# mnastorg/PSI-GNN

Hardware: AMD Instinct MI355X
Metric: fixed-point edges/sec (E' x Broyden iterations/sec) on 1M-node Poisson mesh (higher is better)
Workload: dtype f32

## Files before the change

### psi-gnn_amd/csrc/solver.hip

```cpp
#include "vec_helpers.h"
#include "internal.h"
#include "solver_shapes.h"
#include <stdlib.h>
#include <math.h>
#include <algorithm>
#include <vector>

struct Status {
  int32_t n_iter;
  int32_t done;
  int32_t prot_break;
  int32_t stop_reason;
  int32_t lowest_step;
  int32_t cur;
  int32_t low;
  int32_t nxt;
  double lowest_rel, lowest_abs_at;
  double rel0;
  double abs0;
  int32_t lowest_step_abs;
  int32_t stop_abs;
  double s, beta;
};

#define RB 256
static_assert(shapes::THREADS == TB && sizeof(Status) == shapes::STATUS_BYTES, "solver_shapes.h sizes the launches and the status block");
struct psignn_broyden {
  const psignn_plan* plan = nullptr;
  int64_t M = 0;
  int seq_len = D;
  int thr = 0;
  int keep_trace = 0;
  shapes::BroydenShape shape;
  float* jpart = nullptr;
  float *U = nullptr, *V = nullptr;
  float* xbuf = nullptr;
  float* gbuf[2] = {nullptr, nullptr};
  float *upd = nullptr, *fx = nullptr, *fwork = nullptr;
  float* lwork = nullptr;
  int64_t lwork_floats = 0;
  float* nrm_part = nullptr;
  float* part2 = nullptr;
  int a_ready = 0, a_from = 0;
  float* parta = nullptr;
  float *h0p = nullptr, *prbp = nullptr, *nrmp = nullptr;
  float* part = nullptr;
  float* coef = nullptr;
  Status* st = nullptr;
  double *rel_trace = nullptr, *abs_trace = nullptr;
  Status* h_st = nullptr;
  size_t bytes = 0;
  int ext_iter = 0;
  int hist = 0;
  int stop_abs = 0;
  int64_t size_hint = 0;
  int plan_order = 1;
};

__global__ void k_init_status(Status* st, double* rel_trace, double* abs_trace, int thr, int stop_abs = 0) {
  if (threadIdx.x == 0 && blockIdx.x == 0) {
    st->abs0 = 0.0; st->lowest_step_abs = 0; st->stop_abs = stop_abs;
    st->n_iter = 0; st->done = 0; st->prot_break = 0; st->stop_reason = 0; st->lowest_step = 0;
    st->cur = 0; st->low = 0; st->nxt = 1;
    st->lowest_rel = 1e8; st->lowest_abs_at = 1e8; st->rel0 = 0.0; st->s = 0.0; st->beta = 0.0;
  }
  for (int i = blockIdx.x * blockDim.x + threadIdx.x; i < thr; i += gridDim.x * blockDim.x) {
    rel_trace[i] = 0.0;
    abs_trace[i] = 0.0;
  }
}

template <int VEC>
__global__ __launch_bounds__(TB) void k_begin(int64_t M, const float* __restrict__ x0, const float* __restrict__ fx0,
                                              float* __restrict__ xb, float* __restrict__ gx, float* __restrict__ upd) {
  int64_t e0 = elem0<VEC>();
  if (e0 >= M) return;
// ... 254 lines not shown
  for (int j = 0; j < k; ++j) {
    float u[VEC];
    float sa = 0.f;
    if (act) {
      ldv_stream<VEC>(U + (int64_t)j * ld, e0, M, u);
#pragma unroll
      for (int i = 0; i < VEC; ++i) sa = fmaf(dx[i], u[i], sa);
    }
    sa = wave_sum(sa);
    const int q = j & 63;
    if (lead) sh.v[0][wv][q] = sa;
    if (q == 63 || j == k - 1) {
      float* const rows[1] = {rowb + (j - q)};
      stash_flush<1>(sh, q + 1, rows);
    }
  }
}

template <int VEC>
__global__ __launch_bounds__(TB) void k_sweep_u1(int64_t M, int k, const Status* __restrict__ st, const float* __restrict__ U,
                                                 const float* __restrict__ dxv, float* __restrict__ part, int ldp, int64_t ld) {
  sweep_u1_body<VEC>(M, k, st, U, dxv, part, ldp, ld);
}
template <int VEC>
__global__ __launch_bounds__(TB) void k_sweep_u1_bf16(int64_t M, int k, const Status* __restrict__ st, const __bf16* __restrict__ U,
                                                      const float* __restrict__ dxv, float* __restrict__ part, int ldp, int64_t ld) {
  sweep_u1_body<VEC, __bf16>(M, k, st, U, dxv, part, ldp, ld);
}

__device__ __forceinline__ void reduce_a_check_body(Status* st, const float* __restrict__ part, int nrows, int ldp, int thr, int k,
                                                    float* __restrict__ coef, const float* __restrict__ nrm_part, int nn,
                                                    double* __restrict__ rel_trace, double* __restrict__ abs_trace,
                                                    double eps, int seq_len, int keep_trace, double* sh,
                                                    const float* __restrict__ parta = nullptr, int nrows4 = 0, int a_from = 1 << 30) {
  if (blockIdx.y == RA) {
    if (blockIdx.x == 0) check_block(st, nrm_part, nn, rel_trace, abs_trace, eps, thr, seq_len, keep_trace, sh);
    return;
  }
  const int done = st->done;
  const int j = blockIdx.x, r = blockIdx.y;
  if (j >= k) return;
  const float* col = j >= a_from ? parta + (j - a_from) : part + j;
  const int n = j >= a_from ? nrows4 : nrows;
  const int64_t stride = j >= a_from ? PARTA_LD : ldp;
  const int lo = (int)((int64_t)n * r / RA), hi = (int)((int64_t)n * (r + 1) / RA);
  const double s = block_sum_col(col + (int64_t)lo * stride, hi - lo, stride, sh);
  if (threadIdx.x == 0 && !done) coef[(3 + r) * thr + j] = (float)s;
}
__global__ __launch_bounds__(RB) void k_reduce_a_check(Status* st, const float* __restrict__ part, int nrows, int ldp, int thr, int k,
                                                       float* __restrict__ coef, const float* __restrict__ nrm_part, int nn,
                                                       double* __restrict__ rel_trace, double* __restrict__ abs_trace,
                                                       double eps, int seq_len, int keep_trace, const float* __restrict__ parta,
                                                       int nrows4, int a_from) {
  __shared__ double sh[RB];
  reduce_a_check_body(st, part, nrows, ldp, thr, k, coef, nrm_part, nn, rel_trace, abs_trace, eps, seq_len, keep_trace, sh, parta, nrows4, a_from);
}

template <int VEC, class P = float>
__device__ __forceinline__ void sweep_v_body(int64_t M, int k, const Status* __restrict__ st, P* __restrict__ V,
                                             const float* __restrict__ dxv, const float* __restrict__ dgv,
                                             const float* __restrict__ gv, const float* __restrict__ coef,
                                             float* __restrict__ part, int64_t pstride, int ldp, float* __restrict__ part2, int nblk, int64_t ld,
                                             int thr) {
  __shared__ PairStash<2> sh;
  if (__builtin_amdgcn_readfirstlane(st->done)) return;
  int64_t e0 = elem0<VEC>();
  float dg[VEC], g[VEC], av[VEC];
  const bool act = e0 < M;
  if (act) {
    ldv<VEC>(dxv, e0, M, av);
    ldv<VEC>(dgv, e0, M, dg);
    ldv<VEC>(gv, e0, M, g);
#pragma unroll
    for (int i = 0; i < VEC; ++i) dg[i] = g[i] - dg[i];
#pragma unroll
    for (int i = 0; i < VEC; ++i) av[i] = -av[i];
  } else {
#pragma unroll
    for (int i = 0; i < VEC; ++i) dg[i] = g[i] = av[i] = 0.f;
  }
  const int wv = threadIdx.x >> 6;
  const int lane = threadIdx.x & 63;
  const bool lead = lane == 0;
  float* rowb = part + (int64_t)blockIdx.x * ldp;
  float cw = 0.f;
  auto step = [&](const int j, const float* v) {
    const int q = j & 63;
    if (q == 0) {
// ... 289 lines not shown
  float ccv = 0.f, cbv = 0.f;
  if (lane < NK) {
    ccv = coef[thr + j_keep0 + lane];
    cbv = coef[2 * thr + j_keep0 + lane];
  }
  const float sv = rfl((float)st->s), beta = rfl((float)st->beta);
#pragma unroll
  for (int q = 0; q < NK; ++q) {
    const float cc = __builtin_bit_cast(float, __builtin_amdgcn_readlane(__builtin_bit_cast(int, ccv), q));
    const float cb = __builtin_bit_cast(float, __builtin_amdgcn_readlane(__builtin_bit_cast(int, cbv), q));
    a1[0] = fmaf(-cc, kp[q].x, a1[0]); a1[1] = fmaf(-cc, kp[q].y, a1[1]); a1[2] = fmaf(-cc, kp[q].z, a1[2]); a1[3] = fmaf(-cc, kp[q].w, a1[3]);
    a2[0] = fmaf(-cb, kp[q].x, a2[0]); a2[1] = fmaf(-cb, kp[q].y, a2[1]); a2[2] = fmaf(-cb, kp[q].z, a2[2]); a2[3] = fmaf(-cb, kp[q].w, a2[3]);
  }
#pragma unroll
  for (int i = 0; i < 4; ++i) {
    float q = a1[i] / sv;
    q = (q != q) ? 0.f : q;
    a1[i] = q;
    a2[i] = fmaf(-q, beta, a2[i]);
  }
  st4_so_stream(U + (int64_t)k * ld, off, make_float4(a1[0], a1[1], a1[2], a1[3]));
  st4_so(upd, off, make_float4(a2[0], a2[1], a2[2], a2[3]));
#pragma unroll
  for (int q = 0; q < NK; ++q) {
    float sa = fmaf(kp[q].x, a2[0], fmaf(kp[q].y, a2[1], fmaf(kp[q].z, a2[2], kp[q].w * a2[3])));
    sa = wave_sum(sa);
    if (lead) ua[q] = sa;
  }
  float sa = fmaf(a1[0], a2[0], fmaf(a1[1], a2[1], fmaf(a1[2], a2[2], a1[3] * a2[3])));
  sa = wave_sum(sa);
  if (lead) ua[NK] = sa;
}

template <int KB>
__device__ __forceinline__ void sweep_u2r_body(int64_t M, int k, const Status* __restrict__ st, float* __restrict__ U,
                                               float* __restrict__ upd, const float* __restrict__ dgv,
                                               const float* __restrict__ gv, const float* __restrict__ coef, int thr,
                                               float* __restrict__ part, int64_t ld, int j_keep0) {
  __shared__ float ua[TB / 64][PARTA_LD];
  if (__builtin_amdgcn_readfirstlane(st->done)) return;
  const int tid = threadIdx.x;
  const int64_t e0 = elem0<4>();
  const int wv = __builtin_amdgcn_readfirstlane(tid >> 6);
  const bool lead = (tid & 63) == 0;
  const int64_t wave_e0 = ((int64_t)blockIdx.x * TB + (int64_t)__builtin_amdgcn_readfirstlane(tid & ~63)) * 4;
  if (wave_e0 + 256 <= M) {
    uint32_t off = ((blockIdx.x * (uint32_t)TB + ((uint32_t)tid & ~63u)) * 4u + ((uint32_t)tid & 63u) * 4u) * 4u;
    asm volatile("" : "+v"(off));
    float a1[4], a2[4];
#define U2R_CASE(n, first) case (n): u2r_kept<(n) < 0 ? 0 : (n), first>(a1, a2, k, st, U, upd, dgv, gv, coef, thr, ua[wv], ld, j_keep0, off, lead); break;
    if (j_keep0 == 0) {
      switch (k) {
        U2R_CASE(KB - 8, true) U2R_CASE(KB - 7, true) U2R_CASE(KB - 6, true) U2R_CASE(KB - 5, true) U2R_CASE(KB - 4, true)
        U2R_CASE(KB - 3, true) U2R_CASE(KB - 2, true) U2R_CASE(KB - 1, true) U2R_CASE(KB, true)
        default: break;
      }
    } else {
      {
        const float4 x = ld4_so(upd, off), go = ld4_so(dgv, off), g = ld4_so(gv, off);
        a1[0] = x.x + (g.x - go.x); a1[1] = x.y + (g.y - go.y); a1[2] = x.z + (g.z - go.z); a1[3] = x.w + (g.w - go.w);
        a2[0] = g.x; a2[1] = g.y; a2[2] = g.z; a2[3] = g.w;
      }
      int j = 0;
      const int lane8 = tid & 7, half = (tid >> 3) & 1;
      for (; j + U2D_UNROLL <= j_keep0; j += U2D_UNROLL) {
        float4 u[U2D_UNROLL];
        const float* Uj = U + (int64_t)j * ld;
        asm volatile("" : "+v"(off));
        const float cv = coef[(1 + half) * thr + j + lane8];
#pragma unroll
        for (int q = 0; q < U2D_UNROLL; ++q) u[q] = ld4_so_stream(Uj + (int64_t)q * ld, off);
#pragma unroll
// ... 38 lines not shown
#pragma unroll
      for (int i = 0; i < 4; ++i) {
        a1[i] = fmaf(-cc, u[i], a1[i]);
        a2[i] = fmaf(-cb, u[i], a2[i]);
      }
    }
    if (in) {
      const float sv = (float)st->s, beta = (float)st->beta;
#pragma unroll
      for (int i = 0; i < 4; ++i) {
        float q = a1[i] / sv;
        q = (q != q) ? 0.f : q;
        a1[i] = q;
        a2[i] = fmaf(-q, beta, a2[i]);
      }
      stv<4>(U + (int64_t)k * ld, e0, M, a1);
      stv<4>(upd, e0, M, a2);
#pragma unroll
      for (int i = 0; i < 4; ++i)
        if (e0 + i >= M) a1[i] = a2[i] = 0.f;
    }
    for (int jj = j_keep0; jj <= k; ++jj) {
      float u[4] = {a1[0], a1[1], a1[2], a1[3]};
      if (jj < k) {
        u[0] = u[1] = u[2] = u[3] = 0.f;
        if (in) ldv<4>(U + (int64_t)jj * ld, e0, M, u);
      }
      float sa = fmaf(u[0], a2[0], fmaf(u[1], a2[1], fmaf(u[2], a2[2], u[3] * a2[3])));
      sa = wave_sum(sa);
      if (lead) ua[wv][jj - j_keep0] = sa;
    }
  }
  __syncthreads();
  if (tid <= k - j_keep0) part[(int64_t)blockIdx.x * PARTA_LD + tid] = (ua[0][tid] + ua[1][tid]) + (ua[2][tid] + ua[3][tid]);
}
template <int KB> struct U2RWaves { static constexpr int value = KB <= 8 ? 8 : KB <= 16 ? 5 : 4; };
template <int KB>
__global__ __launch_bounds__(TB, U2RWaves<KB>::value) void k_sweep_u2r(int64_t M, int k, const Status* __restrict__ st, float* __restrict__ U,
                                                                      float* __restrict__ upd, const float* __restrict__ dgv,
                                                                      const float* __restrict__ gv, const float* __restrict__ coef, int thr,
                                                                      float* __restrict__ part, int64_t ld, int j_keep0) {
  sweep_u2r_body<KB>(M, k, st, U, upd, dgv, gv, coef, thr, part, ld, j_keep0);
}

template <int VEC>
__device__ __forceinline__ void axpy_finish(int64_t M, int k, int64_t e0, float* av, float* a1, float* a2, const float* dg,
                                            const float* g, float* __restrict__ U, float* __restrict__ V,
                                            float* __restrict__ upd, float& p1, float& p2, int64_t ld) {
#pragma unroll
  for (int i = 0; i < VEC; ++i) {
    p1 = fmaf(av[i], dg[i], p1);
    av[i] = (av[i] != av[i]) ? 0.f : av[i];
    p2 = fmaf(av[i], g[i], p2);
  }
  stv<VEC>(V + (int64_t)k * ld, e0, M, av);
  stv<VEC>(U + (int64_t)k * ld, e0, M, a1);
  stv<VEC>(upd, e0, M, a2);
}

template <int VEC>
__device__ __forceinline__ void axpy_body(int64_t M, int k, const Status* __restrict__ st, float* __restrict__ U,
                                             float* __restrict__ V, float* __restrict__ upd ,
                                             const float* __restrict__ dgv, const float* __restrict__ gv,
                                             const float* __restrict__ coef, int thr, float* __restrict__ part, int npart,
                                             int jstride, float* __restrict__ jpart, int64_t ld, const bool split) {
  if (st->done) return;
  const int j0 = blockIdx.y * jstride, j1 = min(k, j0 + jstride);
  int64_t e0 = elem0<VEC>();
  float p1 = 0.f, p2 = 0.f;
// ... 251 lines not shown
}

static inline int sel_off_cur() { return offsetof(Status, cur) / 4; }
static inline int sel_off_low() { return offsetof(Status, low) / 4; }
static inline int sel_off_nxt() { return offsetof(Status, nxt) / 4; }

static inline __bf16* bf16_pairs(float* p) { return reinterpret_cast<__bf16*>(p); }

using shapes::update_chain;

struct SingleTarget {
  psignn_broyden* s;
  hipStream_t st;
  float* gnew;
  const float* gold;
  int np;
  const shapes::BroydenShape& size_class() const { return s->shape; }
  void bytes(int64_t b) const { PROF_BYTES(b); }
  int64_t vec_bytes() const { return s->M * 4; }
  int pair_elem_bytes() const { return s->hist ? 2 : 4; }
  int& a_ready() { return s->a_ready; }
  int& a_from() { return s->a_from; }
  int groups(int k) const { return (s->shape.jgroups > 1 && k >= 4 * s->shape.jgroups) ? s->shape.jgroups : 1; }
  bool combine_due(int, int G) const { return G > 1; }
  unsigned gu() const { return (unsigned)s->shape.nblk_u; }

  void sweep_u1(int n1) {
    if (s->hist) VLAUNCH("k_sweep_u1_bf16", st, s->shape.vec_u, k_sweep_u1_bf16, (gu(), TB, 0, st), s->M, n1, s->st, bf16_pairs(s->U), s->upd, s->part, s->shape.ldp, s->shape.ld);
    else VLAUNCH("k_sweep_u1", st, s->shape.vec_u, k_sweep_u1, (gu(), TB, 0, st), s->M, n1, s->st, s->U, s->upd, s->part, s->shape.ldp, s->shape.ld);
  }
  void reduce_a_check(int kd, double eps, int a_from) {
    LAUNCH("k_reduce_check", st, (k_reduce_a_check<<<dim3(std::max(kd, 1), RA + 1), RB, 0, st>>>(
        s->st, s->part, s->shape.nblk_u, s->shape.ldp, s->thr, kd, s->coef, s->nrm_part, np, s->rel_trace, s->abs_trace, eps, s->seq_len, s->keep_trace,
        s->parta, s->shape.nblk4, a_from)));
  }
  void sweep_v(int k) {
    if (s->hist) VLAUNCH("k_sweep_v_bf16", st, s->shape.vec_u, k_sweep_v_bf16, (gu(), TB, 0, st), s->M, k, s->st, bf16_pairs(s->V), s->upd, gold, gnew, s->coef, s->part, s->shape.pstride, s->shape.ldp, s->part2, s->shape.nblk_u, s->shape.ld, s->thr);
    else VLAUNCH("k_sweep_v", st, s->shape.vec_u, k_sweep_v, (gu(), TB, 0, st), s->M, k, s->st, s->V, s->upd, gold, gnew, s->coef, s->part, s->shape.pstride, s->shape.ldp, s->part2, s->shape.nblk_u, s->shape.ld, s->thr);
  }
  void reduce_cb(int k) {
    LAUNCH("k_reduce_cb", st, (k_reduce_cb<<<dim3(std::max(k, 1), 3), RB, 0, st>>>(s->st, s->part, s->shape.nblk_u, s->shape.pstride, s->shape.ldp, s->thr, k, s->coef, s->part2, s->shape.nblk_u)));
  }
  template <int KB>
  void sweep_u2r(int k, int keep0) {
    LAUNCH("k_sweep_u2d", st, (k_sweep_u2r<KB><<<(unsigned)s->shape.nblk4, TB, 0, st>>>(s->M, k, s->st, s->U, s->upd, gold, gnew, s->coef, s->thr, s->parta, s->shape.ld, keep0)));
  }
  void sweep_u2d(int k, int keep0, size_t lds) {
    LAUNCH("k_sweep_u2d", st, (k_sweep_u2d<<<(unsigned)s->shape.nblk4, TB, lds, st>>>(s->M, k, s->st, s->U, s->upd, gold, gnew, s->coef, s->thr, s->parta, s->shape.ld, keep0)));
  }
  void sweep_u2(int k) {
    if (s->hist) VLAUNCH("k_sweep_u2_bf16", st, s->shape.vec_u, k_sweep_u2_bf16, (gu(), TB, 0, st), s->M, k, s->st, bf16_pairs(s->U), s->upd, gold, gnew, s->coef, s->thr, s->shape.ld);
    else VLAUNCH("k_sweep_u2", st, s->shape.vec_u, k_sweep_u2, (gu(), TB, 0, st), s->M, k, s->st, s->U, s->upd, gold, gnew, s->coef, s->thr, s->shape.ld);
  }
  void dots(int kd, int G) {
    VLAUNCH("k_dots", st, s->shape.vec, k_dots, (dim3((unsigned)s->shape.nblk, G), TB, 0, st), s->M, kd, s->st, s->U, s->V, s->upd, gold, gnew, s->part, s->shape.pstride, s->shape.ldp, (int)cdiv(kd, G), s->shape.ld);
  }
  void reduce_check(int kd, double eps) {
    LAUNCH("k_reduce_check", st, (k_reduce_check<<<dim3(std::max(kd, 1), 4), RB, 0, st>>>(
        s->st, s->part, s->shape.nblk, s->shape.pstride, s->shape.ldp, s->thr, kd, s->coef, s->nrm_part, np, s->rel_trace, s->abs_trace, eps, s->seq_len, s->keep_trace)));
  }
  void axpy(int k, int G, bool own_width) {
    const int nb = own_width ? s->shape.nblk_ax : s->shape.nblk;
    VLAUNCH("k_axpy", st, own_width ? s->shape.vec_ax : s->shape.vec, k_axpy, (dim3((unsigned)nb, G), TB, 0, st), s->M, k, s->st, s->U, s->V, s->upd, gold, gnew, s->coef, s->thr, s->part, nb, (int)cdiv(std::max(k, 1), G), s->jpart, s->shape.ld);
  }
  void combine(int k, int G) {
    VLAUNCH("k_axpy_combine", st, s->shape.vec, k_axpy_combine, ((unsigned)s->shape.nblk, TB, 0, st), s->M, k, G, s->st, s->jpart, s->U, s->V, s->upd, gold, gnew, s->part, s->shape.nblk, s->shape.ld);
  }
  void final_pass(int k, bool own_width) {
    const int nb = own_width ? s->shape.nblk_ax : s->shape.nblk;
    VLAUNCH("k_final", st, own_width ? s->shape.vec_ax : s->shape.vec, k_final, ((unsigned)nb, TB, 0, st), s->M, k, s->st, s->U, s->upd, s->shape.ld, s->part, nb);
  }
};

static void launch_update(psignn_broyden* s, int k, double eps, hipStream_t st, int fused_npart = 0) {
  SingleTarget t{s, st, s->gbuf[(k + 1) & 1], s->gbuf[k & 1], fused_npart ? fused_npart : s->shape.nblk};
  if (!fused_npart) {
    PROF_BYTES(3 * (int64_t)s->M * 4);
    VLAUNCH("k_resid", st, s->shape.vec, k_resid, ((unsigned)s->shape.nblk, TB, 0, st), s->M, s->st, s->xbuf, s->fx, t.gnew, s->nrm_part, s->shape.nblk);
  }
  update_chain(t, k, eps);
// ... 191 lines not shown
    const shapes::BroydenShape& c = sv[m]->shape;
    sh.max_g = std::max(sh.max_g, c.nblk);
    sh.max_ga = std::max(sh.max_ga, c.nblk_ax);
    sh.max_gu = std::max(sh.max_gu, c.nblk_u);
    sh.max_g4 = std::max(sh.max_g4, c.nblk4);
    sh.max_G = std::max(sh.max_G, c.jgroups);
    sh.Mtot4 += sv[m]->M * 4;
  }
  return sh;
}

struct ShardTarget {
  const psignn_broyden* s0;
  BatchShape& sh;
  const BatchDesc* dd;
  hipStream_t st;
  const shapes::BroydenShape& size_class() const { return s0->shape; }
  void bytes(int64_t b) const { PROF_BYTES(b); }
  int64_t vec_bytes() const { return sh.Mtot4; }
  int pair_elem_bytes() const { return 4; }
  int& a_ready() { return sh.a_ready; }
  int& a_from() { return sh.a_from_next; }
  int groups(int k) const { return (sh.max_G > 1 && k >= 4 * sh.max_G) ? sh.max_G : 1; }
  bool combine_due(int k, int) const { return sh.max_G > 1 && k >= 4 * 2; }
  dim3 grid(int x, int y = 1) const { return dim3((unsigned)x, (unsigned)y, (unsigned)sh.n); }

  void sweep_u1(int n1) { VLAUNCH("k_sweep_u1", st, s0->shape.vec_u, kb_sweep_u1, (grid(sh.max_gu), TB, 0, st), dd, n1); }
  void reduce_a_check(int kd, double eps, int a_from) {
    LAUNCH("k_reduce_check", st, (kb_reduce_a_check<<<grid(std::max(kd, 1), RA + 1), RB, 0, st>>>(dd, kd, eps, a_from)));
  }
  void sweep_v(int k) { VLAUNCH("k_sweep_v", st, s0->shape.vec_u, kb_sweep_v, (grid(sh.max_gu), TB, 0, st), dd, k, k & 1); }
  void reduce_cb(int k) { LAUNCH("k_reduce_cb", st, (kb_reduce_cb<<<grid(std::max(k, 1), 3), RB, 0, st>>>(dd, k))); }
  template <int KB>
  void sweep_u2r(int k, int keep0) { LAUNCH("k_sweep_u2d", st, (kb_sweep_u2r<KB><<<grid(sh.max_g4), TB, 0, st>>>(dd, k, keep0, k & 1))); }
  void sweep_u2d(int k, int keep0, size_t lds) { LAUNCH("k_sweep_u2d", st, (kb_sweep_u2d<<<grid(sh.max_g4), TB, lds, st>>>(dd, k, keep0, k & 1))); }
  void sweep_u2(int k) { VLAUNCH("k_sweep_u2", st, s0->shape.vec_u, kb_sweep_u2, (grid(sh.max_gu), TB, 0, st), dd, k, k & 1); }
  void dots(int kd, int) { VLAUNCH("k_dots", st, s0->shape.vec, kb_dots, (grid(sh.max_g, sh.max_G), TB, 0, st), dd, kd, kd & 1); }
  void reduce_check(int kd, double eps) { LAUNCH("k_reduce_check", st, (kb_reduce_check<<<grid(std::max(kd, 1), 4), RB, 0, st>>>(dd, kd, eps))); }
  void axpy(int k, int, bool own_width) {
    if (own_width) VLAUNCH("k_axpy", st, s0->shape.vec_ax, kb_axpy, (grid(sh.max_ga), TB, 0, st), dd, k, 1, k & 1);
    else VLAUNCH("k_axpy", st, s0->shape.vec, kb_axpy, (grid(sh.max_g, sh.max_G), TB, 0, st), dd, k, 0, k & 1);
  }
  void combine(int k, int) { VLAUNCH("k_axpy_combine", st, s0->shape.vec, kb_axpy_combine, (grid(sh.max_g), TB, 0, st), dd, k, k & 1); }
  void final_pass(int k, bool own_width) {
    VLAUNCH("k_final", st, own_width ? s0->shape.vec_ax : s0->shape.vec, kb_final, (grid(own_width ? sh.max_ga : sh.max_g), TB, 0, st), dd, k, own_width ? 1 : 0);
  }
};

static void fill_desc(const psignn_broyden* s, BatchDesc& d) {
  const shapes::BroydenShape& c = s->shape;
  d.M = s->M; d.ld = c.ld; d.nblk = c.nblk; d.npart = c.npart; d.nblk_ax = c.nblk_ax; d.jgroups = c.jgroups;
  d.thr = s->thr; d.seq_len = s->seq_len; d.keep_trace = s->keep_trace; d.n_tiles = (int)s->plan->n_tiles;
  d.st = reinterpret_cast<int32_t*>(s->st);
  d.U = s->U; d.V = s->V; d.xbuf = s->xbuf; d.g0 = s->gbuf[0]; d.g1 = s->gbuf[1]; d.upd = s->upd; d.part = s->part; d.coef = s->coef;
  d.nrm_part = s->nrm_part; d.jpart = s->jpart; d.rel_trace = s->rel_trace; d.abs_trace = s->abs_trace;
  d.ctx = s->plan->d_ctx; d.h0p = s->h0p; d.prbp = s->prbp;
  d.part2 = s->part2; d.nblk_u = c.nblk_u; d.npart_u = c.npart_u;
  d.parta = s->parta; d.nblk4 = c.nblk4; d.pad_ = 0; d.pstride = c.pstride;
  d.fx = s->fx; d.xcopy = s->h0p; d.pad2_ = 0;
}
static int shard_all_done(const BatchDesc* d_descs, int n, int32_t* d_done, int32_t* h_done, hipStream_t st) {
  kb_all_done<<<1, 64, 0, st>>>(d_descs, n, offsetof(Status, done) / 4, d_done);
  HIP_TRY(hipMemcpyAsync(h_done, d_done, 4, hipMemcpyDeviceToHost, st));
  HIP_TRY(hipStreamSynchronize(st));
  return PSIGNN_OK;
}
static int shard_finish(int n, psignn_broyden_t** sv, float* const* d_results, psignn_solve_info_t* infos, double* const* h_rel,
                        double* const* h_abs, hipStream_t st) {
  int rc = PSIGNN_OK;
  for (int m = 0; m < n && rc == PSIGNN_OK; ++m)
    rc = finish(sv[m], d_results ? d_results[m] : nullptr, infos ? &infos[m] : nullptr, h_rel ? h_rel[m] : nullptr,
                h_abs ? h_abs[m] : nullptr, st);
  return rc;
}

extern "C" int psignn_broyden_batchable(int n, psignn_broyden_t* const* sv) {
  if (n <= 0 || !sv || !sv[0] || !sv[0]->plan) return 0;
  const psignn_broyden* s0 = sv[0];
  for (int m = 0; m < n; ++m) {
    const psignn_broyden* s = sv[m];
    if (!s || !s->plan || !s->plan->tiled || s->plan->mixed != s0->plan->mixed) return 0;
    if (s->hist) return 0;
    if (!s->shape.same_size_class(s0->shape)) return 0;
  }
  return 1;
}

extern "C" int psignn_broyden_solve_batch(int n, psignn_broyden_t** sv, const float* W, int nl, const float* const* h0,
                                          const float* const* prb, const float* const* nrm, double eps, int poll_every,
                                          float* const* d_results, psignn_solve_info_t* infos, double* const* h_rel,
                                          double* const* h_abs, void* stream) {
  ARG_CHECK(n > 0 && sv && W && h0 && prb, "bad arguments");
  ARG_CHECK(nl == 1, "the batched solver runs single-layer blocks");
  ARG_CHECK(psignn_broyden_batchable(n, sv),
            "batched solve: tiled plans of one boundary-condition family and one size class, fp32 pair history (psignn_broyden_batchable)");
  for (int m = 0; m < n; ++m) {
    ARG_CHECK(h0[m] && prb[m], "NULL argument");
    ARG_CHECK(!sv[m]->plan->mixed || (nrm && nrm[m]), "mixed plans need unit normals");
  }
  hipStream_t st = (hipStream_t)stream;
  if (poll_every <= 0) poll_every = 8;
  const psignn_broyden* s0 = sv[0];
  BatchShape sh = shard_shape(n, sv);
  int max_rows = 0, n_slots = 0;
  int64_t bf_tot = 0;
  std::vector<BatchDesc> hd(n);
  int rc;
  for (int m = 0; m < n; ++m) {
    psignn_broyden* s = sv[m];
    const psignn_plan* p = s->plan;
    max_rows = std::max(max_rows, p->max_rows);
    bf_tot += (p->mixed ? 8 * D + 22 : 8 * D + 9) * p->N + 20 * p->Ep + 8 * s->M;
    s->plan_order = 1;
    k_init_status<<<4, TB, 0, st>>>(s->st, s->rel_trace, s->abs_trace, s->thr, s->stop_abs);
    if ((rc = psignn_plan_permute(p, h0[m], D, s->h0p, 1, st))) return rc;
// ... 227 lines not shown
    VLAUNCH("k_addv_resid", st, s0->shape.vec, kb_addv_resid, (gv, TB, 0, st), d_descs.get(), it & 1);
    update_chain(t, it, eps);
    if ((it + 1) % poll_every == 0 || it + 1 == thr) {
      if ((rc = shard_all_done(d_descs.get(), n, d_done.get(), h_done.get(), st))) return rc;
      if (*h_done.get()) break;
    }
  }
  return shard_finish(n, sv, d_results, infos, h_rel, h_abs, st);
}
#endif


extern "C" int psignn_broyden_get_iterate(const psignn_broyden_t* s, int i, float* d_dst, void* stream) {
  ARG_CHECK(s && d_dst, "NULL argument");
  ARG_CHECK(s->keep_trace, "solver was created without keep_trace");
  ARG_CHECK(i >= 0 && i <= s->thr, "iterate index out of range");
  if (s->plan && s->plan_order) {
    VPLAIN(s->shape.vec, k_copy_sel, ((unsigned)s->shape.nblk, TB, 0, (hipStream_t)stream), s->M, s->xbuf, nullptr, i, s->fx);
    return psignn_plan_permute(s->plan, s->fx, D, d_dst, 0, stream);
  }
  VPLAIN(s->shape.vec, k_copy_sel, ((unsigned)s->shape.nblk, TB, 0, (hipStream_t)stream), s->M, s->xbuf, nullptr, i, d_dst);
  HIP_TRY(hipGetLastError());
  return PSIGNN_OK;
}

__global__ __launch_bounds__(TB) void k_widen_bf16(int64_t M, const __bf16* __restrict__ src, float* __restrict__ dst) {
  for (int64_t i = (int64_t)blockIdx.x * TB + threadIdx.x; i < M; i += (int64_t)gridDim.x * TB) dst[i] = (float)src[i];
}

extern "C" int psignn_broyden_get_pair(const psignn_broyden_t* s, int j, int which, float* d_dst, void* stream) {
  ARG_CHECK(s && d_dst, "NULL argument");
  ARG_CHECK(which >= 0 && which <= 3, "which: 0 = U_j, 1 = V_j, 2 = the current update vector, 3 = partials of the folded sweep");
  if (which == 3) {
    HIP_TRY(hipMemcpyAsync(d_dst, s->parta, (size_t)std::min<int64_t>(s->M, (int64_t)s->shape.nblk4 * PARTA_LD) * 4, hipMemcpyDeviceToDevice, (hipStream_t)stream));
    return PSIGNN_OK;
  }
  ARG_CHECK(which == 2 || (j >= 0 && j < s->thr), "pair index out of range");
  if (s->hist && which != 2) {
    const __bf16* row = bf16_pairs(which ? s->V : s->U) + (int64_t)j * s->shape.ld;
    float* dst = s->plan && s->plan_order ? s->fx : d_dst;
    k_widen_bf16<<<(unsigned)std::min<int64_t>(cdiv(s->M, TB), 4096), TB, 0, (hipStream_t)stream>>>(s->M, row, dst);
    HIP_TRY(hipGetLastError());
    if (s->plan && s->plan_order) return psignn_plan_permute(s->plan, s->fx, D, d_dst, 0, stream);
    return PSIGNN_OK;
  }
  const float* row = which == 2 ? s->upd : (which ? s->V : s->U) + (int64_t)j * s->shape.ld;
  if (s->plan && s->plan_order) {
    HIP_TRY(hipMemcpyAsync(s->fx, row, (size_t)s->M * 4, hipMemcpyDeviceToDevice, (hipStream_t)stream));
    return psignn_plan_permute(s->plan, s->fx, D, d_dst, 0, stream);
  }
  HIP_TRY(hipMemcpyAsync(d_dst, row, (size_t)s->M * 4, hipMemcpyDeviceToDevice, (hipStream_t)stream));
  return PSIGNN_OK;
}

extern "C" int psignn_broyden_ext_begin(psignn_broyden_t* s, const float* d_x0, const float* d_fx0, void* stream) {
  ARG_CHECK(s && d_x0 && d_fx0, "NULL argument");
  hipStream_t st = (hipStream_t)stream;
  k_init_status<<<4, TB, 0, st>>>(s->st, s->rel_trace, s->abs_trace, s->thr, s->stop_abs);
  VPLAIN(s->shape.vec, k_begin, ((unsigned)s->shape.nblk, TB, 0, st), s->M, d_x0, d_fx0, s->xbuf, s->gbuf[0], s->upd);
  s->ext_iter = 0;
  HIP_TRY(hipGetLastError());
  return PSIGNN_OK;
}
extern "C" int psignn_broyden_ext_next_x(psignn_broyden_t* s, float* d_x_new, void* stream) {
  ARG_CHECK(s && d_x_new, "NULL argument");
  VPLAIN(s->shape.vec, k_xnext, ((unsigned)s->shape.nblk, TB, 0, (hipStream_t)stream), s->M, s->st, s->xbuf, s->upd, d_x_new);
  HIP_TRY(hipGetLastError());
// ... 83 lines not shown
```

### psi-gnn_amd/csrc/solver_shapes.h

```cpp
#pragma once
#include <stddef.h>
#include <stdint.h>
#include <stdlib.h>
#include <algorithm>

#include "workspace.h"

namespace shapes {
constexpr int THREADS = 256;
constexpr int WAVE = 64;
constexpr size_t STATUS_BYTES = 88;
constexpr int64_t VEC16_MIN = (int64_t)3 << 18;
inline int64_t cdiv(int64_t a, int64_t b) { return (a + b - 1) / b; }
}

#define PARTA_LD 32
#define RA 8
#define U2R_KB_MAX 24
#define U2D_LDS_KMAX (PARTA_LD - 1)
static_assert(U2R_KB_MAX + 1 <= PARTA_LD, "the register fold's kept pairs must fit a partials row");

namespace shapes {
struct Knob {
  bool set = false;
  int64_t v = 0;
};
struct Knobs {
  Knob vec16_min;
  Knob jgroups;
  Knob vec_ax4;
  Knob uvu;
  Knob u2d_lds;
  Knob u2d_kmax;
  Knob u2d_keep;
};
inline Knobs knobs_from_env() {
  Knobs k;
  auto num = [](const char* name, Knob& kn, bool wide) {
    if (const char* e = getenv(name)) kn = {true, wide ? (int64_t)atoll(e) : (int64_t)atoi(e)};
  };
  num("PSIGNN_VEC16_MIN", k.vec16_min, true);
  num("PSIGNN_JGROUPS", k.jgroups, false);
  num("PSIGNN_VEC_AX4", k.vec_ax4, false);
  num("PSIGNN_UVU", k.uvu, false);
  if (const char* e = getenv("PSIGNN_U2D_FORM")) k.u2d_lds = {true, (e[0] == 'l' || e[0] == 'L') ? 1 : 0};
  num("PSIGNN_U2D_KMAX", k.u2d_kmax, false);
  num("PSIGNN_U2D_KEEP", k.u2d_keep, false);
  return k;
}

struct VecShape {
  int vec, nblk, npart;
  int64_t ld;
};
inline VecShape vec_shape(int64_t n_elems, int64_t width_elems, int64_t vec16_min = VEC16_MIN) {
  const int vec = width_elems >= vec16_min ? 16 : 4;
  const int nblk = (int)cdiv(n_elems, (int64_t)vec * THREADS);
  return {vec, nblk, nblk * (THREADS / WAVE), (n_elems + 63) / 64 * 64};
}

struct BroydenShape {
  int thr = 0;
  int vec = 16;
  int nblk = 0, npart = 0;
  int vec_ax = 0, nblk_ax = 0;
  int jgroups = 1;
  int uvu = 0;
  int vec_u = 0, nblk_u = 0, npart_u = 0;
  int u2d_kmax = 0, nblk4 = 0;
  int u2d_keep = 0;
  int u2d_reg = 1;
  int nn_cap = 0;
  int ldp = 0;
  int64_t pstride = 0;
  int64_t ld = 0;
  struct Bytes {
    size_t U, V, xbuf, gbuf0, gbuf1, upd, fx, part, parta, coef, st, nrm_part, part2, rel_trace, abs_trace;
    size_t jpart, fwork, h0p, prbp, nrmp;
    size_t total() const {
      return U + V + xbuf + gbuf0 + gbuf1 + upd + fx + part + parta + coef + st + nrm_part + part2 + rel_trace + abs_trace + jpart + fwork +
             h0p + prbp + nrmp;
    }
  } bytes = {};

  bool wants_big_lds() const { return u2d_kmax > 0 && !u2d_reg; }
  void cap_to_default_lds() {
    u2d_kmax = std::min(u2d_kmax, 15);
    u2d_keep = std::min(u2d_keep, 15);
  }
  bool same_size_class(const BroydenShape& b) const {
    return vec == b.vec && vec_ax == b.vec_ax && uvu == b.uvu && vec_u == b.vec_u && thr == b.thr && u2d_kmax == b.u2d_kmax &&
           u2d_keep == b.u2d_keep && u2d_reg == b.u2d_reg;
  }
};

inline BroydenShape broyden_shape(int64_t M, int64_t size_hint, int thr, int hist, int keep_trace, int64_t plan_nodes, int64_t n_tiles,
                                  const Knobs& kn) {
  BroydenShape s;
  s.thr = thr;
  const int64_t eff = std::max<int64_t>(M, size_hint);
  const VecShape v = vec_shape(M, eff, kn.vec16_min.set ? kn.vec16_min.v : VEC16_MIN);
  s.vec = v.vec;
  s.nblk = v.nblk;
  const int64_t eff_blk = cdiv(eff, (int64_t)s.vec * THREADS);
  s.jgroups = eff_blk >= 768 ? 1 : (int)std::min<int64_t>(8, cdiv(768, eff_blk));
  const bool short_shard = size_hint > M && s.vec == 16 && s.nblk < 512;
  if (short_shard) s.jgroups = 4;
  if (kn.jgroups.set) s.jgroups = std::max(1, std::min(8, (int)kn.jgroups.v));
  s.npart = v.npart;
  s.vec_ax = s.vec;
  s.nblk_ax = s.nblk;
  s.nblk4 = (int)cdiv(M, (int64_t)4 * THREADS);
  if (kn.vec_ax4.set ? (kn.vec_ax4.v != 0 && s.vec == 16) : (s.vec == 16 && s.jgroups > 1 && (short_shard || s.nblk4 >= 512))) {
    s.vec_ax = 4;
    s.nblk_ax = s.nblk4;
  }
  const bool long_form = s.vec == 16 && s.jgroups == 1 && s.vec_ax == 16;
  if (long_form) {
    s.uvu = 1; s.vec_u = 16; s.nblk_u = s.nblk;
  } else if (s.vec_ax == 4 && s.vec == 16) {
    s.uvu = 1; s.vec_u = 4; s.nblk_u = s.nblk_ax;
  }
  if (kn.uvu.set && kn.uvu.v == 0) s.uvu = 0;
  if (hist) {
    s.uvu = 1;
    s.vec_u = long_form ? 16 : 4;
    s.nblk_u = (int)cdiv(M, (int64_t)s.vec_u * THREADS);
  }
  s.npart_u = s.nblk_u * (THREADS / WAVE);
  const bool fold_ok = s.uvu != 0;
  const bool reg_reaches = M < ((int64_t)1 << 30);
  s.u2d_reg = (kn.u2d_lds.set ? !kn.u2d_lds.v : cdiv(eff, (int64_t)4 * THREADS) >= 2048) && reg_reaches;
  const int kmax_cap = s.u2d_reg ? U2R_KB_MAX : U2D_LDS_KMAX;
  s.u2d_kmax = fold_ok ? 24 : 0;
  if (kn.u2d_kmax.set) s.u2d_kmax = fold_ok ? std::max(0, std::min(kmax_cap, (int)kn.u2d_kmax.v)) : 0;
  s.u2d_keep = s.u2d_kmax > 0 ? 16 : 0;
  if (kn.u2d_keep.set) s.u2d_keep = s.u2d_kmax > 0 ? std::max(0, std::min(s.u2d_kmax, (int)kn.u2d_keep.v)) : 0;
  if (hist) s.u2d_kmax = s.u2d_keep = 0;
  s.nn_cap = std::max<int>(std::max(s.nblk, s.nblk_ax), (int)n_tiles);
  s.ldp = (thr + 63) / 64 * 64;
  s.pstride = (int64_t)std::max(std::max(s.nblk, s.nblk_u), std::max(s.nblk_ax, 1)) * s.ldp;
  s.ld = hist ? (M + 127) / 128 * 128 : v.ld;
  const size_t m4 = (size_t)M * 4, t = (size_t)thr, nx = keep_trace ? t + 2 : 3;
  const size_t pair = t * (size_t)s.ld * (hist ? 2 : 4);
  const bool split_axpy = s.jgroups > 1 && s.vec_ax == s.vec;
  const size_t N = (size_t)plan_nodes;
  s.bytes = {pair, pair, nx * m4, m4, m4, m4, m4, 3 * (size_t)s.pstride * 4 + 16, (size_t)s.nblk4 * PARTA_LD * 4 + 16,
             (3 + RA) * t * 4 + 16, STATUS_BYTES, 2 * (size_t)s.nn_cap * 4 + 16, 2 * (size_t)std::max(s.nblk, s.nblk_u) * 4 + 16, t * 8 + 8,
             t * 8 + 8,
             split_axpy ? (size_t)s.jgroups * 3 * m4 : 0, N ? (size_t)ws::f_total(plan_nodes) * 4 : 0, N ? m4 : 0, N * 3 * 4, N * 2 * 4};
  return s;
}

template <class Target>
static void update_chain(Target& t, int k, double eps) {
  const BroydenShape& c = t.size_class();
  const int thr = c.thr;
  const int64_t vb = t.vec_bytes();
  const int64_t pe = vb / 4 * t.pair_elem_bytes();
  const int kd = k >= thr ? 0 : k;
  const bool last = k + 1 >= thr;
  if (c.uvu) {
    if (k == 0) t.a_ready() = 0;
    const int a_from = t.a_ready() ? t.a_from() : kd;
    const int n1 = std::min(a_from, kd);
    if (n1 > 0) {
      t.bytes(n1 * pe + vb);
      t.sweep_u1(n1);
    }
    t.reduce_a_check(kd, eps, a_from);
    t.a_ready() = 0;
    if (k >= thr) return;
    t.bytes(last ? 0 : (k + 1) * pe + 3 * vb);
    t.sweep_v(k);
    t.reduce_cb(k);
    const int keep0 = k <= c.u2d_kmax ? 0 : k - c.u2d_keep;
    if (c.u2d_kmax > 0 && (k <= c.u2d_kmax || c.u2d_keep > 0) && !last) {
      t.bytes((k + 1) * pe + 4 * vb);
      const int nk = k - keep0;
      if (!c.u2d_reg) t.sweep_u2d(k, keep0, (size_t)std::max(nk, 1) * THREADS * 16);
      else if (nk <= 8) t.template sweep_u2r<8>(k, keep0);
      else if (nk <= 16) t.template sweep_u2r<16>(k, keep0);
      else t.template sweep_u2r<24>(k, keep0);
      t.a_ready() = 1;
      t.a_from() = keep0;
    } else {
      t.bytes(last ? 0 : (k + 1) * pe + 4 * vb);
      t.sweep_u2(k);
    }
    return;
  }
  const int G = t.groups(k);
  if (kd > 0) {
    t.bytes((2 * kd + 3) * vb);
    t.dots(kd, G);
  }
  t.reduce_check(kd, eps);
  if (k >= thr) return;
  const bool own_width = c.vec_ax != c.vec;
  const int Ga = own_width ? 1 : G;
  t.bytes(last ? 0 : (2 * k + (Ga > 1 ? 3 * Ga : 6)) * vb);
  t.axpy(k, Ga, own_width);
  if (!own_width && t.combine_due(k, G)) {
    t.bytes(last || G <= 1 ? 0 : (3 * G + 6) * vb);
    t.combine(k, G);
  }
  t.bytes(last ? 0 : 4 * vb);
  t.final_pass(k, own_width);
}
}
```

Before: 2.440 billion.

## Widen register-folded U sweep to fuse up to 48 kept Broyden pairs

Adds a wide mode for the register-resident fused U2 sweep. For large meshes it raises the fold cap from 24 to 48 pairs, uses a 64-wide partials pitch and adds KB=32/40/48 template instances with lower occupancy targets. More Broyden iterations can then fold the next step's U dot products into the update sweep, so the separate U1 read pass over the stored pairs is skipped. The cost is more register pressure and lower occupancy in the wide kernels, and the batched path is disabled when wide mode is on.

```diff
diff --git a/psi-gnn_amd/csrc/solver.hip b/psi-gnn_amd/csrc/solver.hip
--- a/psi-gnn_amd/csrc/solver.hip
+++ b/psi-gnn_amd/csrc/solver.hip
@@ -42,6 +42,7 @@
   float* nrm_part = nullptr;
   float* part2 = nullptr;
   int a_ready = 0, a_from = 0;
+  int a_ld = PARTA_LD;
   float* parta = nullptr;
   float *h0p = nullptr, *prbp = nullptr, *nrmp = nullptr;
   float* part = nullptr;
@@ -362,7 +363,8 @@
                                                     float* __restrict__ coef, const float* __restrict__ nrm_part, int nn,
                                                     double* __restrict__ rel_trace, double* __restrict__ abs_trace,
                                                     double eps, int seq_len, int keep_trace, double* sh,
-                                                    const float* __restrict__ parta = nullptr, int nrows4 = 0, int a_from = 1 << 30) {
+                                                    const float* __restrict__ parta = nullptr, int nrows4 = 0, int a_from = 1 << 30,
+                                                    int lda = PARTA_LD ) {
   if (blockIdx.y == RA) {
     if (blockIdx.x == 0) check_block(st, nrm_part, nn, rel_trace, abs_trace, eps, thr, seq_len, keep_trace, sh);
     return;
@@ -372,7 +374,7 @@
   if (j >= k) return;
   const float* col = j >= a_from ? parta + (j - a_from) : part + j;
   const int n = j >= a_from ? nrows4 : nrows;
-  const int64_t stride = j >= a_from ? PARTA_LD : ldp;
+  const int64_t stride = j >= a_from ? lda : ldp;
   const int lo = (int)((int64_t)n * r / RA), hi = (int)((int64_t)n * (r + 1) / RA);
   const double s = block_sum_col(col + (int64_t)lo * stride, hi - lo, stride, sh);
   if (threadIdx.x == 0 && !done) coef[(3 + r) * thr + j] = (float)s;
@@ -381,9 +383,9 @@
                                                        float* __restrict__ coef, const float* __restrict__ nrm_part, int nn,
                                                        double* __restrict__ rel_trace, double* __restrict__ abs_trace,
                                                        double eps, int seq_len, int keep_trace, const float* __restrict__ parta,
-                                                       int nrows4, int a_from) {
+                                                       int nrows4, int a_from, int lda) {
   __shared__ double sh[RB];
-  reduce_a_check_body(st, part, nrows, ldp, thr, k, coef, nrm_part, nn, rel_trace, abs_trace, eps, seq_len, keep_trace, sh, parta, nrows4, a_from);
+  reduce_a_check_body(st, part, nrows, ldp, thr, k, coef, nrm_part, nn, rel_trace, abs_trace, eps, seq_len, keep_trace, sh, parta, nrows4, a_from, lda);
 }
 
 template <int VEC, class P = float>
@@ -739,12 +741,14 @@
   if (lead) ua[NK] = sa;
 }
 
+template <int KB> struct U2RPitch { static constexpr int value = KB + 1 <= PARTA_LD ? PARTA_LD : PARTA_LD_WIDE; };
 template <int KB>
 __device__ __forceinline__ void sweep_u2r_body(int64_t M, int k, const Status* __restrict__ st, float* __restrict__ U,
                                                float* __restrict__ upd, const float* __restrict__ dgv,
                                                const float* __restrict__ gv, const float* __restrict__ coef, int thr,
                                                float* __restrict__ part, int64_t ld, int j_keep0) {
-  __shared__ float ua[TB / 64][PARTA_LD];
+  constexpr int LDA = U2RPitch<KB>::value;
+  __shared__ float ua[TB / 64][LDA];
   if (__builtin_amdgcn_readfirstlane(st->done)) return;
   const int tid = threadIdx.x;
   const int64_t e0 = elem0<4>();
@@ -849,9 +853,9 @@
     }
   }
   __syncthreads();
-  if (tid <= k - j_keep0) part[(int64_t)blockIdx.x * PARTA_LD + tid] = (ua[0][tid] + ua[1][tid]) + (ua[2][tid] + ua[3][tid]);
-}
-template <int KB> struct U2RWaves { static constexpr int value = KB <= 8 ? 8 : KB <= 16 ? 5 : 4; };
+  if (tid <= k - j_keep0) part[(int64_t)blockIdx.x * LDA + tid] = (ua[0][tid] + ua[1][tid]) + (ua[2][tid] + ua[3][tid]);
+}
+template <int KB> struct U2RWaves { static constexpr int value = KB <= 8 ? 8 : KB <= 16 ? 5 : KB <= 24 ? 4 : KB <= 32 ? 3 : 2; };
 template <int KB>
 __global__ __launch_bounds__(TB, U2RWaves<KB>::value) void k_sweep_u2r(int64_t M, int k, const Status* __restrict__ st, float* __restrict__ U,
                                                                       float* __restrict__ upd, const float* __restrict__ dgv,
@@ -1169,7 +1173,7 @@
   void reduce_a_check(int kd, double eps, int a_from) {
     LAUNCH("k_reduce_check", st, (k_reduce_a_check<<<dim3(std::max(kd, 1), RA + 1), RB, 0, st>>>(
         s->st, s->part, s->shape.nblk_u, s->shape.ldp, s->thr, kd, s->coef, s->nrm_part, np, s->rel_trace, s->abs_trace, eps, s->seq_len, s->keep_trace,
-        s->parta, s->shape.nblk4, a_from)));
+        s->parta, s->shape.nblk4, a_from, s->a_ld)));
   }
   void sweep_v(int k) {
     if (s->hist) VLAUNCH("k_sweep_v_bf16", st, s->shape.vec_u, k_sweep_v_bf16, (gu(), TB, 0, st), s->M, k, s->st, bf16_pairs(s->V), s->upd, gold, gnew, s->coef, s->part, s->shape.pstride, s->shape.ldp, s->part2, s->shape.nblk_u, s->shape.ld, s->thr);
@@ -1180,9 +1184,11 @@
   }
   template <int KB>
   void sweep_u2r(int k, int keep0) {
+    s->a_ld = U2RPitch<KB>::value;
     LAUNCH("k_sweep_u2d", st, (k_sweep_u2r<KB><<<(unsigned)s->shape.nblk4, TB, 0, st>>>(s->M, k, s->st, s->U, s->upd, gold, gnew, s->coef, s->thr, s->parta, s->shape.ld, keep0)));
   }
   void sweep_u2d(int k, int keep0, size_t lds) {
+    s->a_ld = PARTA_LD;
     LAUNCH("k_sweep_u2d", st, (k_sweep_u2d<<<(unsigned)s->shape.nblk4, TB, lds, st>>>(s->M, k, s->st, s->U, s->upd, gold, gnew, s->coef, s->thr, s->parta, s->shape.ld, keep0)));
   }
   void sweep_u2(int k) {
@@ -1440,7 +1446,9 @@
   void sweep_v(int k) { VLAUNCH("k_sweep_v", st, s0->shape.vec_u, kb_sweep_v, (grid(sh.max_gu), TB, 0, st), dd, k, k & 1); }
   void reduce_cb(int k) { LAUNCH("k_reduce_cb", st, (kb_reduce_cb<<<grid(std::max(k, 1), 3), RB, 0, st>>>(dd, k))); }
   template <int KB>
-  void sweep_u2r(int k, int keep0) { LAUNCH("k_sweep_u2d", st, (kb_sweep_u2r<KB><<<grid(sh.max_g4), TB, 0, st>>>(dd, k, keep0, k & 1))); }
+  void sweep_u2r(int k, int keep0) {
+    if constexpr (KB <= U2R_KB_NARROW) LAUNCH("k_sweep_u2d", st, (kb_sweep_u2r<KB><<<grid(sh.max_g4), TB, 0, st>>>(dd, k, keep0, k & 1)));
+  }
   void sweep_u2d(int k, int keep0, size_t lds) { LAUNCH("k_sweep_u2d", st, (kb_sweep_u2d<<<grid(sh.max_g4), TB, lds, st>>>(dd, k, keep0, k & 1))); }
   void sweep_u2(int k) { VLAUNCH("k_sweep_u2", st, s0->shape.vec_u, kb_sweep_u2, (grid(sh.max_gu), TB, 0, st), dd, k, k & 1); }
   void dots(int kd, int) { VLAUNCH("k_dots", st, s0->shape.vec, kb_dots, (grid(sh.max_g, sh.max_G), TB, 0, st), dd, kd, kd & 1); }
@@ -1489,6 +1497,7 @@
     const psignn_broyden* s = sv[m];
     if (!s || !s->plan || !s->plan->tiled || s->plan->mixed != s0->plan->mixed) return 0;
     if (s->hist) return 0;
+    if (s->shape.u2d_wide) return 0;
     if (!s->shape.same_size_class(s0->shape)) return 0;
   }
   return 1;
@@ -1782,7 +1791,7 @@
   ARG_CHECK(s && d_dst, "NULL argument");
   ARG_CHECK(which >= 0 && which <= 3, "which: 0 = U_j, 1 = V_j, 2 = the current update vector, 3 = partials of the folded sweep");
   if (which == 3) {
-    HIP_TRY(hipMemcpyAsync(d_dst, s->parta, (size_t)std::min<int64_t>(s->M, (int64_t)s->shape.nblk4 * PARTA_LD) * 4, hipMemcpyDeviceToDevice, (hipStream_t)stream));
+    HIP_TRY(hipMemcpyAsync(d_dst, s->parta, (size_t)std::min<int64_t>(s->M, (int64_t)s->shape.nblk4 * s->shape.parta_ld) * 4, hipMemcpyDeviceToDevice, (hipStream_t)stream));
     return PSIGNN_OK;
   }
   ARG_CHECK(which == 2 || (j >= 0 && j < s->thr), "pair index out of range");
diff --git a/psi-gnn_amd/csrc/solver_shapes.h b/psi-gnn_amd/csrc/solver_shapes.h
--- a/psi-gnn_amd/csrc/solver_shapes.h
+++ b/psi-gnn_amd/csrc/solver_shapes.h
@@ -15,10 +15,12 @@
 }
 
 #define PARTA_LD 32
+#define PARTA_LD_WIDE 64
 #define RA 8
-#define U2R_KB_MAX 24
+#define U2R_KB_NARROW 24
+#define U2R_KB_MAX 48
 #define U2D_LDS_KMAX (PARTA_LD - 1)
-static_assert(U2R_KB_MAX + 1 <= PARTA_LD, "the register fold's kept pairs must fit a partials row");
+static_assert(U2R_KB_NARROW + 1 <= PARTA_LD && U2R_KB_MAX + 1 <= PARTA_LD_WIDE, "the register fold's kept pairs must fit a partials row");
 
 namespace shapes {
 struct Knob {
@@ -33,6 +35,7 @@
   Knob u2d_lds;
   Knob u2d_kmax;
   Knob u2d_keep;
+  Knob u2d_wide;
 };
 inline Knobs knobs_from_env() {
   Knobs k;
@@ -46,6 +49,7 @@
   if (const char* e = getenv("PSIGNN_U2D_FORM")) k.u2d_lds = {true, (e[0] == 'l' || e[0] == 'L') ? 1 : 0};
   num("PSIGNN_U2D_KMAX", k.u2d_kmax, false);
   num("PSIGNN_U2D_KEEP", k.u2d_keep, false);
+  num("PSIGNN_U2D_WIDE", k.u2d_wide, false);
   return k;
 }
 
@@ -70,6 +74,8 @@
   int u2d_kmax = 0, nblk4 = 0;
   int u2d_keep = 0;
   int u2d_reg = 1;
+  int u2d_wide = 0;
+  int parta_ld = PARTA_LD;
   int nn_cap = 0;
   int ldp = 0;
   int64_t pstride = 0;
@@ -90,7 +96,7 @@
   }
   bool same_size_class(const BroydenShape& b) const {
     return vec == b.vec && vec_ax == b.vec_ax && uvu == b.uvu && vec_u == b.vec_u && thr == b.thr && u2d_kmax == b.u2d_kmax &&
-           u2d_keep == b.u2d_keep && u2d_reg == b.u2d_reg;
+           u2d_keep == b.u2d_keep && u2d_reg == b.u2d_reg && u2d_wide == b.u2d_wide;
   }
 };
 
@@ -131,8 +137,10 @@
   const bool fold_ok = s.uvu != 0;
   const bool reg_reaches = M < ((int64_t)1 << 30);
   s.u2d_reg = (kn.u2d_lds.set ? !kn.u2d_lds.v : cdiv(eff, (int64_t)4 * THREADS) >= 2048) && reg_reaches;
-  const int kmax_cap = s.u2d_reg ? U2R_KB_MAX : U2D_LDS_KMAX;
-  s.u2d_kmax = fold_ok ? 24 : 0;
+  s.u2d_wide = s.u2d_reg && fold_ok && !hist && size_hint <= M && (kn.u2d_wide.set ? kn.u2d_wide.v != 0 : s.nblk4 >= 4096);
+  s.parta_ld = s.u2d_wide ? PARTA_LD_WIDE : PARTA_LD;
+  const int kmax_cap = s.u2d_reg ? (s.u2d_wide ? U2R_KB_MAX : U2R_KB_NARROW) : U2D_LDS_KMAX;
+  s.u2d_kmax = fold_ok ? (s.u2d_wide ? U2R_KB_MAX : 24) : 0;
   if (kn.u2d_kmax.set) s.u2d_kmax = fold_ok ? std::max(0, std::min(kmax_cap, (int)kn.u2d_kmax.v)) : 0;
   s.u2d_keep = s.u2d_kmax > 0 ? 16 : 0;
   if (kn.u2d_keep.set) s.u2d_keep = s.u2d_kmax > 0 ? std::max(0, std::min(s.u2d_kmax, (int)kn.u2d_keep.v)) : 0;
@@ -145,7 +153,7 @@
   const size_t pair = t * (size_t)s.ld * (hist ? 2 : 4);
   const bool split_axpy = s.jgroups > 1 && s.vec_ax == s.vec;
   const size_t N = (size_t)plan_nodes;
-  s.bytes = {pair, pair, nx * m4, m4, m4, m4, m4, 3 * (size_t)s.pstride * 4 + 16, (size_t)s.nblk4 * PARTA_LD * 4 + 16,
+  s.bytes = {pair, pair, nx * m4, m4, m4, m4, m4, 3 * (size_t)s.pstride * 4 + 16, (size_t)s.nblk4 * s.parta_ld * 4 + 16,
              (3 + RA) * t * 4 + 16, STATUS_BYTES, 2 * (size_t)s.nn_cap * 4 + 16, 2 * (size_t)std::max(s.nblk, s.nblk_u) * 4 + 16, t * 8 + 8,
              t * 8 + 8,
              split_axpy ? (size_t)s.jgroups * 3 * m4 : 0, N ? (size_t)ws::f_total(plan_nodes) * 4 : 0, N ? m4 : 0, N * 3 * 4, N * 2 * 4};
@@ -181,7 +189,10 @@
       if (!c.u2d_reg) t.sweep_u2d(k, keep0, (size_t)std::max(nk, 1) * THREADS * 16);
       else if (nk <= 8) t.template sweep_u2r<8>(k, keep0);
       else if (nk <= 16) t.template sweep_u2r<16>(k, keep0);
-      else t.template sweep_u2r<24>(k, keep0);
+      else if (nk <= 24) t.template sweep_u2r<24>(k, keep0);
+      else if (nk <= 32) t.template sweep_u2r<32>(k, keep0);
+      else if (nk <= 40) t.template sweep_u2r<40>(k, keep0);
+      else t.template sweep_u2r<48>(k, keep0);
       t.a_ready() = 1;
       t.a_from() = keep0;
     } else {
```

New measurement: 2.453 billion (median of 6 runs). Within noise of the previous version (+0.5%).
